# HaydenFaulkner/VidDet

Hardware: AMD Instinct MI355X
Metric: frames/sec (416x416) yolo3_darknet53 fwd+bwd (higher is better)
Workload: dtype f32; 1 GPU; yolo3_darknet53_coco training, batch 64/GPU, 416x416, fp32, fwd+bwd+SGD-momentum (BASELINE configs[2]; the reference trains with SGD, not Adam); classes=80, global_batch=64, parallelism=dp1, hip_graph=False

## Files before the change

### include/viddet_hip.h

```cpp
#ifndef VIDDET_HIP_H
#define VIDDET_HIP_H

#include <stdint.h>

#ifdef __cplusplus
extern "C" {
#endif

#define VD_OK            0
#define VD_EINVAL       -1
#define VD_ELAUNCH      -2
#define VD_EWORKSPACE   -3

#define VD_MAX_TAPS 27

#define VD_EPI_AFFINE    1
#define VD_EPI_LEAKY     2
#define VD_EPI_RESIDUAL  4
#define VD_MATH_SPLIT    16
#define VD_MATH_BF16     32

#define VD_MATH_F16X2    64
#define VD_MATH_NOHALO   128
#define VD_STORE_BF16    256
#define VD_WGRAD_HALO    512
#define VD_CONV_STREAMK  1024
#define VD_CONV_PARITY4  2048
#define VD_CONV_SPLITK   4096
#define VD_SK_MAX_WG        2048
#define VD_SK_HEADER_BYTES  32768
#define VD_SK_SPLIT_CNT_OFF   4096
#define VD_SK_SPLIT_MAX_TILES 4096
#define VD_SK_TIMEOUT_TICKS 4000
#define VD_AMAX_SLOTS    32
#define VD_AMAX_STRIDE   64
#define VD_AMAX_FLOATS   (VD_AMAX_SLOTS * VD_AMAX_STRIDE)

const char* vd_last_error(void);
int vd_version(void);
#define VD_ABI_VERSION 6
int vd_abi_version(void);
int64_t vd_sizeof_desc(int which);

typedef struct {
    const float* in;
    const float* wp;
    float*       out;
    const float* scale;
    const float* shift;
    const float* residual;
    int32_t N, Hi, Wi, Ci;
    int32_t Hg, Wg;
    int32_t in_stride;
    int32_t T;
    int32_t dy[VD_MAX_TAPS], dx[VD_MAX_TAPS];
// ... 11 lines not shown
    float*  stats_part;
    const float* bs_z;
    const float* bs_scale;
    const float* bs_shift;
    const float* bs_mean;
    const float* bs_invstd;
    float*  bs_part;
    float   bs_slope;
    const float* amax_in;
    const float* amax_w;
    float*  amax_out;
    void*   sk_ws;
    int64_t sk_ws_bytes;
    int32_t par_cin;
    int32_t par_mask;
} vd_conv_desc;

int vd_conv_igemm(const vd_conv_desc* d, void* stream);
int vd_conv_igemm_streamk(const vd_conv_desc* d);
int64_t vd_conv_igemm_streamk_ws_bytes(void);
int vd_conv_igemm_mtiles(const vd_conv_desc* d);

int vd_conv_igemm_bf16(const vd_conv_desc* d, int out_f32, void* stream);
int vd_conv_igemm_bf16_streamk(const vd_conv_desc* d, int out_f32);
int vd_conv_igemm_bf16_mtiles(const vd_conv_desc* d);
int vd_pack_weight_bf16(const float* wp_f32, void* wp_bf16, int Co, int Co_pad, int Ci, int Ci_pad, int T,
                        void* stream);
int vd_stem_im2col_bf16(const float* in, void* col, int N, int H, int W, int nchw, void* stream);

typedef struct {
// ... 67 lines not shown
                    const double* sums2, double count, int64_t M, int C, float slope,
                    float* dx, float* amax_out , void* stream);

typedef struct {
    const float* gamma;
    const float* beta;
    const float* scale;
    int32_t C;
    int32_t pad_;
} vd_guard_item;
int vd_range_guard(const vd_guard_item* items, int n, float thresh, float* ratios, int32_t* flags, void* stream);

int vd_amax_merge(const float* a, const float* b, float* out, void* stream);
int vd_amax(const float* x, int64_t n, float* amax, void* stream);
int vd_amax_segments(const float* base, const int64_t* seg, int nseg, float* amax, void* stream);

int vd_add(const float* a, const float* b, float* out, int64_t n, void* stream);
int vd_fill(float* out, float v, int64_t n, void* stream);
int vd_upsample2x_concat(const float* up, const float* route, float* out,
                         int N, int Ho, int Wo, int Cu, int Cr, void* stream);
int vd_upsample2x_concat_bwd(const float* dout, float* dup, float* droute,
                             int N, int Ho, int Wo, int Cu, int Cr, void* stream);
int vd_nchw_to_nhwc(const float* in, float* out, int N, int C, int H, int W, void* stream);
int vd_preprocess_u8_nhwc(const uint8_t* in, float* out, int64_t npix, void* stream);
int vd_preprocess_u8_nchw(const uint8_t* in, float* out, int N, int H, int W, void* stream);
int vd_temporal_pool(const float* x, float* y, int32_t* argmax, int B, int K, int64_t inner, int type,
                     void* stream);
int vd_temporal_pool_bwd(const float* dy, const int32_t* argmax, float* dx, int B, int K,
                         int64_t inner, int type, void* stream);
int vd_frame_slice(const float* x, float* y, int B, int K, int k0, int kc, int64_t inner, int backward, void* stream);
// ... 58 lines not shown
```

### viddet_amd/csrc/vd_conv.hip

```cpp

#include "vd_conv_igemm.h"

int vd_igemm_sk_dispatch(const vd_conv_desc& d, int tile, hipStream_t s);
int vd_igemm_sk_applies(const vd_conv_desc& d, int tile);
int vd_igemm_par_dispatch(const vd_conv_desc& d, int tile, hipStream_t s);
int vd_igemm_par_tile(int tile);
int vd_igemm_par_bm(int tile);

namespace {

int igemm_resolve_tile(const vd_conv_desc& d) {
    int tile = d.tile;
    if (tile <= 0 || tile > 8) {
        if (d.Co <= 32) tile = 7;
        else if (d.Co <= 64) tile = 6;
        else tile = 2;
    }
    return tile;
}

int igemm_tile_bm(int tile) { return (tile == 4 || tile == 5) ? 64 : 128; }

int igemm_split_resolve_tile(const vd_conv_desc& d) {
    int tile = d.tile;
// ... 530 lines not shown
                }
            }
            v[e] = val;
        }
        reinterpret_cast<f32x4*>(col)[i] = v;
    }
}

int check_taps(int T, const int32_t* dy, const int32_t* dx, int Hi, int Wi) {
    if (T < 1 || T > VD_MAX_TAPS) return 0;
    for (int t = 0; t < T; ++t)
        if (dy[t] < -64 || dy[t] > 64 || dx[t] < -64 || dx[t] > 64) return 0;
    return Hi < 4096 && Wi < 4096;
}

}

extern "C" {

#if VD_STAMP
int vd_debug_stamps_f32(unsigned long long* out) {
    return hipMemcpyFromSymbol(out, HIP_SYMBOL(g_stamps_f32), sizeof(unsigned long long) * 16) == hipSuccess ? 0 : 1;
}
#endif

int vd_conv_igemm(const vd_conv_desc* d, void* stream) {
    VD_REQUIRE(d && d->in && d->wp && d->out, "vd_conv_igemm: null pointer");
    VD_REQUIRE(d->Ci > 0 && d->Ci % 32 == 0, "vd_conv_igemm: Ci=%d must be a positive multiple of 32", d->Ci);
    VD_REQUIRE(d->N > 0 && d->Hg > 0 && d->Wg > 0 && d->Co > 0, "vd_conv_igemm: bad shape");
    VD_REQUIRE(check_taps(d->T, d->dy, d->dx, d->Hi, d->Wi), "vd_conv_igemm: bad tap list (T=%d)", d->T);
    VD_REQUIRE(d->Kfr >= 1 && d->Kfr < 128 && d->N % d->Kfr == 0, "vd_conv_igemm: bad Kfr=%d", d->Kfr);
    VD_REQUIRE((d->flags & VD_CONV_PARITY4) || d->ldo >= d->Co, "vd_conv_igemm: ldo < Co");
    VD_REQUIRE((int64_t)d->N * d->Hi * d->Wi < (1ll << 31), "vd_conv_igemm: input pixel count overflows int32");
    VD_REQUIRE((int64_t)d->N * d->Hg * d->Wg < (1ll << 31), "vd_conv_igemm: GEMM row count overflows int32");
    VD_REQUIRE((d->Hg - 1) * d->out_stride + d->out_oy < d->Ho && (d->Wg - 1) * d->out_stride + d->out_ox < d->Wo,
               "vd_conv_igemm: output grid exceeds output tensor");
    VD_REQUIRE(!(d->flags & VD_EPI_RESIDUAL) || (d->residual && (d->ldr >= d->Co || (d->flags & VD_CONV_PARITY4))), "vd_conv_igemm: residual missing");
    VD_REQUIRE((d->in_scale == nullptr) == (d->in_shift == nullptr), "vd_conv_igemm: in_scale/in_shift mismatch");
    VD_REQUIRE(!d->stats_part || (d->flags & 7) == 0, "vd_conv_igemm: fused BN statistics need a raw (epilogue-free) output");
    VD_REQUIRE(!d->bs_part || (!d->stats_part && !d->in_scale && d->bs_z && d->bs_scale && d->bs_shift && d->bs_mean && d->bs_invstd),
               "vd_conv_igemm: fused BN backward reductions need all five bs_* inputs (and no forward statistics / in-load transform)");
    VD_REQUIRE(!(d->flags & VD_CONV_STREAMK) || !d->sk_ws || ((uintptr_t)d->sk_ws % 16 == 0 && d->sk_ws_bytes >= VD_SK_HEADER_BYTES),
               "vd_conv_igemm: VD_CONV_STREAMK workspace must be 16-byte aligned and hold its header");
    VD_REQUIRE(!(d->flags & VD_MATH_F16X2) || (d->amax_in && d->amax_w && !d->in_scale),
               "vd_conv_igemm: VD_MATH_F16X2 needs amax_in and amax_w (and no in-load transform)");
    hipStream_t s = (hipStream_t)stream;
    if (d->flags & VD_CONV_PARITY4) {
        VD_REQUIRE((d->flags & VD_MATH_F16X2) && !(d->flags & (VD_EPI_AFFINE | VD_EPI_LEAKY)) && !d->stats_part && !d->in_scale,
                   "vd_conv_igemm: VD_CONV_PARITY4 runs in VD_MATH_F16X2 with a residual / bs_* epilogue only");
        VD_REQUIRE(d->T == 4 && d->dy[0] == 0 && d->dx[0] == 0 && d->dy[1] == 0 && d->dx[1] == 1 && d->dy[2] == 1 && d->dx[2] == 0 &&
                   d->dy[3] == 1 && d->dx[3] == 1 && d->in_stride == 1 && d->Hg == d->Hi && d->Wg == d->Wi && d->Kfr == 1,
                   "vd_conv_igemm: VD_CONV_PARITY4 taps are the offsets (0,0) (0,1) (1,0) (1,1) on the gradient's own grid");
        VD_REQUIRE(d->out_stride == 2 && d->Ho == 2 * d->Hg && d->Wo == 2 * d->Wg && d->par_cin >= 32 && d->par_cin % 32 == 0 &&
                   d->Co == 4 * d->par_cin && d->ldo >= d->par_cin && d->ldo % 4 == 0 && (uintptr_t)d->out % 16 == 0 &&
                   (!(d->flags & VD_EPI_RESIDUAL) || (d->ldr % 4 == 0 && (uintptr_t)d->residual % 16 == 0)),
                   "vd_conv_igemm: VD_CONV_PARITY4 geometry (even output, Co = 4 par_cin, aligned rows)");
        VD_REQUIRE(!d->bs_part || (((uintptr_t)d->bs_z | (uintptr_t)d->bs_scale | (uintptr_t)d->bs_shift | (uintptr_t)d->bs_mean |
                                    (uintptr_t)d->bs_invstd) % 16 == 0), "vd_conv_igemm: VD_CONV_PARITY4 bs_* alignment");
        vd_igemm_par_dispatch(*d, vd_igemm_par_tile(d->tile), s);
        VD_CHECK_LAUNCH("vd_conv_igemm/parity4");
        return VD_OK;
    }
    if (d->in_scale) dispatch_igemm<true>(*d, s);
    else dispatch_igemm<false>(*d, s);
    VD_CHECK_LAUNCH("vd_conv_igemm");
    return VD_OK;
}

int vd_conv_igemm_streamk(const vd_conv_desc* d) {
    if (!d || !(d->flags & VD_CONV_STREAMK) || !(d->flags & VD_MATH_F16X2)) return 0;
    return vd_igemm_sk_applies(*d, igemm_split_resolve_tile(*d));
}

int64_t vd_conv_igemm_streamk_ws_bytes(void) {
    return (int64_t)VD_SK_HEADER_BYTES + (int64_t)device_cus() * 256 * 256 * 4;
}

int vd_conv_igemm_mtiles(const vd_conv_desc* d) {
    if (!d) return 0;
    const int64_t M = (int64_t)d->N * d->Hg * d->Wg;
// ... 137 lines not shown
```

### viddet_amd/csrc/vd_conv_igemm.h

```cpp
#pragma once
#include "vd_common.h"
#include "vd_wgrad_halo.h"
#include <stdlib.h>

namespace {


#ifndef VD_WG_REMAP
#define VD_WG_REMAP 1
#endif
#ifndef VD_KORDER
#define VD_KORDER 1
#endif
#ifndef VD_SETPRIO
#define VD_SETPRIO 1
#endif
#ifndef VD_PROBE
#define VD_PROBE 0
#endif
#ifndef VD_PD
#define VD_PD 3
#endif
#ifndef VD_BNT
#define VD_BNT 0
// ... 97 lines not shown
template <> struct Terms<2> { static constexpr int N = 3; static constexpr int QA[6] = {1, 0, 0, 0, 0, 0}, QB[6] = {0, 1, 0, 0, 0, 0}; };
template <> struct Terms<1> { static constexpr int N = 1; static constexpr int QA[6] = {0, 0, 0, 0, 0, 0}, QB[6] = {0, 0, 0, 0, 0, 0}; };

__device__ __forceinline__ unsigned udiv_rcp(unsigned n, unsigned d, unsigned rcp) {
    unsigned q = d == 1u ? n : __umulhi(n, rcp);
    q -= (q * d > n) ? 1u : 0u;
    return q;
}

struct RowInfo {
    int64_t off;
    unsigned mask;
};

template <int WM, int WN, int TM, int TN, bool XF, bool SP, bool M16 = false, bool BS = false, int NPL = 3, bool HALO = false, bool SK = false,
          bool PAR = false>
__global__ __launch_bounds__(WM * WN * 64, ((!SP && WM * WN == 8) ? 4 : ((SP && WM * WN == 4) ? 2 : 1))) void k_conv_igemm(const vd_conv_desc p, const int64_t zd_in, const int64_t zd_w, const int sk_lds_flag, const int sk_timeout) {
    static_assert(NPL == 3 || ((NPL == 1 || NPL == 2) && SP), "planes");
    static_assert(!SK || (NPL == 2 && VD_KORDER && !VD_KROT && !XF), "stream-K: the fp16-split tiles, taps-innermost K order");
    static_assert(!PAR || (NPL == 2 && !HALO && !SK && VD_KORDER && !VD_KROT), "parity-fused data gradient: fp16-split tiles, generic loop");
    static_assert(NPL != 2 || !XF, "the fp16 split needs the max-abs of the operand it splits: no in-load transform");
    static_assert(!HALO || (NPL == 2 && WM * WN == 8 && WN * TN * 32 >= 64), "the halo loop exists for the 8-wave fp16-split tiles");
    constexpr int SP_ROWB = NPL * 64;
    constexpr int NTERM = Terms<NPL>::N;
    static_assert(!M16 || SP, "the 16x16x32 shape exists for the bf16 operands of the split arithmetic");
    constexpr int BM = WM * TM * 32, BN = WN * TN * 32;
    constexpr int NT = WM * WN * 64;
    constexpr int RPP = NT / 8;
    constexpr bool BHALF = BN < RPP;
    constexpr int AP = BM / RPP, BP = BHALF ? 1 : BN / RPP;
    static_assert(WM * WN == 4 || WM * WN == 8, "4 or 8 waves");
    static_assert(BM % RPP == 0 && (BHALF || BN % RPP == 0), "tile vs loader");
    static_assert(!BHALF || SP, "the half-populated weight pass exists for the split-math tiles");
    extern __shared__ __attribute__((aligned(16))) float smem[];
    float* As = smem;
    float* Bs = smem + 2 * BM * LDS_LD;
// ... 16 lines not shown
        const int tg0 = g * tq + (g < tr ? g : tr), tgn = tq + (g < tr ? 1 : 0);
        const int64_t U = (int64_t)tgn * upt;
        const int64_t ub = U * j / gs, ue = U * (j + 1) / gs;
        sk_brem = (int)(ub % upt);
        sk_erem = (int)(ue % upt);
        const int tb = (int)(ub / upt), te = (int)(ue / upt);
        sk_tfirst = tg0 + tb;
        sk_t0 = sk_tfirst + (sk_brem ? 1 : 0);
        sk_nwhole = te - (tb + (sk_brem ? 1 : 0));
        if (sk_nwhole < 0) sk_nwhole = 0;
        sk_tlast = tg0 + te;
        sk_nitems = (sk_erem ? 1 : 0) + sk_nwhole + (sk_brem ? 1 : 0);
        sk_me = gbase + j;
    }
    float amx = 0.f;

    int sexp_a = 0, sexp_b = 0;
    float scl_a = 1.f, scl_b = 1.f;
    if (NPL == 2) {
        sexp_a = vd_f16_scale_exp(vd_amax_read(p.amax_in));
        sexp_b = vd_f16_scale_exp(vd_amax_read(p.amax_w));
        scl_a = __uint_as_float((unsigned)(127 + sexp_a) << 23);
        scl_b = __uint_as_float((unsigned)(127 + sexp_b) << 23);
    }

    STAMP(0);
    const int tlane = (int)(threadIdx.x & 63) < p.T ? (int)(threadIdx.x & 63) : 0;
    const int tap_dy = p.dy[tlane], tap_dx = p.dx[tlane], tap_dz = p.dz[tlane];
    const unsigned rcp_w = 0xFFFFFFFFu / (unsigned)p.Wg + 1u, rcp_h = 0xFFFFFFFFu / (unsigned)p.Hg + 1u;

// ... 138 lines not shown
#pragma unroll
                for (int e = 0; e < 4; ++e) {
                    float t = v[e] * sc[e] + sh[e];
                    t = t > 0.f ? t : t * p.in_slope;
                    v[e] = ok ? t : 0.f;
                }
            }
            ra[i] = v;
        }
        const int64_t koff = (int64_t)t_tap * p.Ci + c0;
#pragma unroll
        for (int i = 0; i < BP; ++i) {
            const int64_t o = boff[i] + koff;
            const int64_t sel = (boff[i] >= 0 && !(VD_PROBE & 16)) ? o : zd_w;
#if VD_BNT
            rb[i] = __builtin_nontemporal_load(reinterpret_cast<const f32x4*>(p.wp + sel));
#else
            rb[i] = *reinterpret_cast<const f32x4*>(p.wp + sel);
#endif
        }
#if VD_KORDER
        ++t_tap;
        if (t_tap >= p.T) {
            t_tap = 0;
            c0 += BK;
            if (VD_KROT && c0 >= p.Ci) c0 = 0;
        }
        tap_soff = tap_off(t_tap);
#else
        c0 += BK;
        if (c0 >= p.Ci) {
            c0 = 0;
            ++t_tap;
// ... 7 lines not shown
            const int c = (tid & 7) >> 1, half = (tid & 1) << 3;
            const int oh = ((c ^ key) << 4) + half, ol = (((4 + c) ^ key) << 4) + half;
            char* a3 = As3 + buf * BM * SP_ROWB;
            char* b3 = Bs3 + buf * BN * SP_ROWB;
#pragma unroll
            for (int i = 0; i < AP; ++i) {
                uint2 h, l;
                split2(ra[i], scl_a, h, l);
                char* r = a3 + (lrow + RPP * i) * SP_ROWB;
                *reinterpret_cast<uint2*>(r + oh) = h;
                *reinterpret_cast<uint2*>(r + ol) = l;
            }
#pragma unroll
            for (int i = 0; i < BP; ++i) {
                if (BHALF && lrow >= BN) break;
                uint2 h, l;
                split2(rb[i], scl_b, h, l);
                char* r = b3 + (lrow + RPP * i) * SP_ROWB;
                *reinterpret_cast<uint2*>(r + oh) = h;
                *reinterpret_cast<uint2*>(r + ol) = l;
            }
            return;
        }
        if (SP) {
            const int wkey = M16 ? 2 * ((lrow >> 3) & 1) : ((lrow >> 2) & 3);
            const int wsl = ((((tid & 7) >> 1) ^ wkey) << 4) + ((tid & 1) << 3);
            char* a3 = As3 + buf * BM * SP_ROWB + wsl;
            char* b3 = Bs3 + buf * BN * SP_ROWB + wsl;
#pragma unroll
            for (int i = 0; i < AP; ++i) {
                uint2 h, m, l;
                char* r = a3 + (lrow + RPP * i) * SP_ROWB;
                if (NPL == 3) {
// ... 182 lines not shown
            return *reinterpret_cast<const f32x4*>(p.in + sel);
        };
        auto hstore = [&](const f32x4 v, int c, int s) {
            const int ro_ = (c & 1) * ABUF + (((hvalid >> s) & 1u) ? s * 8192 : hsink);
            uint2 h, l;
            split2(v, scl_a, h, l);
            *reinterpret_cast<uint2*>(Ah + ro_ + hl0) = h;
            *reinterpret_cast<uint2*>(Ah + ro_ + hl1) = l;
        };
        int bt = 0, bc0 = cbeg * BK;
        auto gloadB = [&](f32x4 (&rb)[BP]) {
            const int64_t koff = (int64_t)bt * p.Ci + bc0;
#pragma unroll
            for (int i = 0; i < BP; ++i) {
                const int64_t sel = boff[i] >= 0 ? boff[i] + koff : zd_w;
                rb[i] = *reinterpret_cast<const f32x4*>(p.wp + sel);
            }
            if (++bt >= HT) { bt = 0; bc0 += BK; }
        };
        auto lstoreB = [&](int buf, const f32x4 (&rb)[BP]) {
            const int key = f16x2_key<M16>(lrow);
            const int oh = ((hcs ^ key) << 4) + hhalf, ol = (((4 + hcs) ^ key) << 4) + hhalf;
#pragma unroll
            for (int i = 0; i < BP; ++i) {
                uint2 h, l;
                split2(rb[i], scl_b, h, l);
                char* r = Bh + (buf * BN + lrow + RPP * i) * 128;
                *reinterpret_cast<uint2*>(r + oh) = h;
                *reinterpret_cast<uint2*>(r + ol) = l;
            }
        };
        const int lsel = M16 ? (lane >> 4) : (lane >> 5);
        auto hrows = [&](int (&av)[NRB], int abuf, int tap) {
            const int ro = __builtin_amdgcn_readlane(tap_ro, tap);
#pragma unroll
            for (int b = 0; b < NRB; ++b) {
                const int j = ((amask[b] >> tap) & 1u) ? jbase[b] + ro : ZROW;
                av[b] = abuf * ABUF + j * 128 + ((f16x2_key<M16>(j) ^ lsel) << 4);
            }
        };
        const int swz = f16x2_key<M16>(lane & (RBS - 1));
        auto fragsA = [&](v4i (&fa)[NRB][2], const int (&av)[NRB], int kc) {
// ... 625 lines not shown
    int lds = lds_fixed;
    if (HALO) {
        const int64_t hb = halo_lds_bytes(BM, BN, d.Wi);
        lds = hb > lds_epi ? (int)hb : lds_epi;
    }
    int64_t nblk = vd_cdiv((int64_t)d.N * d.Hg * d.Wg, BM) * vd_cdiv(d.Co, BN);
    int sk_flag_off = 0;
    if (SK) {
        const int G = streamk_grid(d, BM, BN, (SP && WM * WN == 4) ? 2 : 1);
        lds = (lds + 15) & ~15;
        if (G == 0 || lds + 16 > 160 * 1024) return 1;
        sk_flag_off = lds;
        lds += 16;
        nblk = G;
    }
    static bool attr_done = false;
    auto kfn = k_conv_igemm<WM, WN, TM, TN, XF, SP, M16, BS, NPL, HALO, SK, PAR>;
    if (!attr_done) {
        (void)hipFuncSetAttribute(reinterpret_cast<const void*>(kfn), hipFuncAttributeMaxDynamicSharedMemorySize,
                                  HALO ? 160 * 1024 : lds_fixed + (SK ? 16 : 0));
        attr_done = true;
    }
    const float* zp = zero_page();
    const int64_t zd_in = zp - d.in, zd_w = zp - d.wp;
    static const int sk_timeout = getenv("VD_SK_TIMEOUT_TICKS") ? atoi(getenv("VD_SK_TIMEOUT_TICKS")) : VD_SK_TIMEOUT_TICKS;
    hipLaunchKernelGGL(kfn, dim3((unsigned)nblk), dim3(WM * WN * 64), lds, s, d, zd_in, zd_w, sk_flag_off, sk_timeout);
    return 0;
}

}
```

### viddet_amd/lib.py

```python
import ctypes as C
import os

_HERE = os.path.dirname(os.path.abspath(__file__))
LIB_PATH = os.environ.get("VD_LIB") or os.path.join(_HERE, "csrc", "libviddet_hip.so")

ABI_VERSION = 6
VD_MAX_TAPS = 27
EPI_AFFINE, EPI_LEAKY, EPI_RESIDUAL = 1, 2, 4
MATH_SPLIT = 16
MATH_BF16 = 32
MATH_F16X2 = 64
MATH_NOHALO = 128
STORE_BF16 = 256
WGRAD_HALO = 512
CONV_STREAMK = 1024
CONV_SPLITK = 4096
CONV_PARITY4 = 2048
SK_HEADER_BYTES = 32768
AMAX_SLOTS, AMAX_STRIDE = 32, 64
AMAX_FLOATS = AMAX_SLOTS * AMAX_STRIDE

_fp = C.c_void_p


# ... 2 lines not shown
        ("in_", _fp), ("wp", _fp), ("out", _fp), ("scale", _fp), ("shift", _fp), ("residual", _fp),
        ("N", C.c_int32), ("Hi", C.c_int32), ("Wi", C.c_int32), ("Ci", C.c_int32),
        ("Hg", C.c_int32), ("Wg", C.c_int32), ("in_stride", C.c_int32), ("T", C.c_int32),
        ("dy", C.c_int32 * VD_MAX_TAPS), ("dx", C.c_int32 * VD_MAX_TAPS), ("dz", C.c_int32 * VD_MAX_TAPS),
        ("Kfr", C.c_int32),
        ("Ho", C.c_int32), ("Wo", C.c_int32), ("Co", C.c_int32),
        ("out_stride", C.c_int32), ("out_oy", C.c_int32), ("out_ox", C.c_int32),
        ("ldo", C.c_int32), ("ldr", C.c_int32), ("flags", C.c_int32), ("slope", C.c_float),
        ("in_scale", _fp), ("in_shift", _fp), ("in_slope", C.c_float), ("tile", C.c_int32),
        ("stats_part", _fp),
        ("bs_z", _fp), ("bs_scale", _fp), ("bs_shift", _fp), ("bs_mean", _fp), ("bs_invstd", _fp), ("bs_part", _fp),
        ("bs_slope", C.c_float),
        ("amax_in", _fp), ("amax_w", _fp), ("amax_out", _fp),
        ("sk_ws", _fp), ("sk_ws_bytes", C.c_int64),
        ("par_cin", C.c_int32), ("par_mask", C.c_int32),
    ]


class WgradDesc(C.Structure):
    _fields_ = [
        ("in_", _fp), ("dout", _fp), ("dwp", _fp),
        ("N", C.c_int32), ("Hi", C.c_int32), ("Wi", C.c_int32), ("Ci", C.c_int32),
        ("Hg", C.c_int32), ("Wg", C.c_int32), ("Co", C.c_int32), ("ldd", C.c_int32),
        ("in_stride", C.c_int32), ("T", C.c_int32),
        ("dy", C.c_int32 * VD_MAX_TAPS), ("dx", C.c_int32 * VD_MAX_TAPS), ("dz", C.c_int32 * VD_MAX_TAPS),
        ("Kfr", C.c_int32), ("splits", C.c_int32),
        ("in_scale", _fp), ("in_shift", _fp), ("in_slope", C.c_float), ("flags", C.c_int32),
        ("amax_in", _fp), ("amax_dout", _fp),
    ]

# ... 37 lines not shown
    "vd_bn_stats": (_i, [_p, _i64, _i, _p, _p, _i64, _p]),
    "vd_bn_sum_partials_ws_bytes": (_i64, [_i, _i]),
    "vd_bn_sum_partials": (_i, [_p, _i, _i, _p, _p, _i64, _p]),
    "vd_bn_finalize": (_i, [_p, _d, _i, _p, _p, _f, _f, _p, _p, _p, _p, _p, _p, _p]),
    "vd_bn_sum_finalize": (_i, [_p, _i, _i, _p, _d, _p, _p, _f, _f, _p, _p, _p, _p, _p, _p, _p, _i64, _p]),
    "vd_bn_sum_param_grads": (_i, [_p, _i, _i, _p, _p, _p, _p, _i64, _p]),
    "vd_bn_fold_eval": (_i, [_p, _p, _p, _p, _f, _i, _p, _p, _p]),
    "vd_bn_apply_leaky": (_i, [_p, _p, _p, _p, _p, _i64, _i, _f, _p, _p]),
    "vd_bn_bwd_reduce": (_i, [_p, _p, _p, _p, _p, _p, _i64, _i, _f, _p, _p, _i64, _p]),
    "vd_bn_param_grads": (_i, [_p, _i, _p, _p, _p]),
    "vd_bn_bwd_apply": (_i, [_p, _p, _p, _p, _p, _p, _p, _d, _i64, _i, _f, _p, _p, _p]),
    "vd_range_guard": (_i, [_p, _i, _f, _p, _p, _p]),
    "vd_amax": (_i, [_p, _i64, _p, _p]),
    "vd_amax_segments": (_i, [_p, _p, _i, _p, _p]),
    "vd_amax_merge": (_i, [_p, _p, _p, _p]),
    "vd_add": (_i, [_p, _p, _p, _i64, _p]),
    "vd_fill": (_i, [_p, _f, _i64, _p]),
    "vd_upsample2x_concat": (_i, [_p, _p, _p, _i, _i, _i, _i, _i, _p]),
    "vd_upsample2x_concat_bwd": (_i, [_p, _p, _p, _i, _i, _i, _i, _i, _p]),
    "vd_nchw_to_nhwc": (_i, [_p, _p, _i, _i, _i, _i, _p]),
    "vd_stem_conv_blocks": (_i, [_i, _i, _i]),
    "vd_stem_conv": (_i, [_p, _p, _p, _i, _i, _i, _i, _p, _p, C.c_float, _i, _i, _p, _p]),
    "vd_stem_conv_c32_bf16": (_i, [_p, _p, _p, _p, C.c_float, C.POINTER(ConvDesc), _p]),
    "vd_stem_wgrad_ws_bytes": (_i64, [_i, _i, _i]),
    "vd_stem_wgrad": (_i, [_p, _p, _i, _p, _i, _i, _i, _p, _i64, _p]),
    "vd_preprocess_u8_nhwc": (_i, [_p, _p, _i64, _p]),
    "vd_preprocess_u8_nchw": (_i, [_p, _p, _i, _i, _i, _p]),
    "vd_temporal_pool": (_i, [_p, _p, _p, _i, _i, _i64, _i, _p]),
    "vd_temporal_pool_bwd": (_i, [_p, _p, _p, _i, _i, _i64, _i, _p]),
    "vd_temporal_cat": (_i, [_p, _p, _i, _i, _i64, _i, _i, _p]),
# ... 68 lines not shown
```

### viddet_amd/model.py

```python
import ctypes as C
import math
import re
from collections import OrderedDict

import numpy as np
import torch

from . import lib as L
from . import ops
from .lib import ConvDesc, WgradDesc, EPI_AFFINE, EPI_LEAKY, EPI_RESIDUAL
from .ops import round_up, fwd_taps, dgrad_plans

from .consts import ANCHORS, STRIDES, BN_EPS, BN_MOMENTUM, LEAKY_SLOPE


class Slot:

    def __init__(self):
        self.value = None


class Program:

    def __init__(self):
# ... 116 lines not shown
            return None
        return str(torch.cuda.get_device_properties(torch.cuda.current_device()).gcnArchName).split(":")[0]

    def _read_file(self):
        import ast
        import json
        import os
        out = {}
        p = self.path()
        if p is None or not os.path.exists(p):
            return out
        try:
            doc = json.load(open(p))
            if doc.get("library") not in (None, self.library_id()):
                return out
            arch = self.device_arch()
            if arch is not None and doc.get("device") not in (None, arch):
                return out
            for k, v in doc.get("entries", {}).items():
                out[ast.literal_eval(k)] = tuple(v) if isinstance(v, list) else v
        except (OSError, ValueError, SyntaxError) as e:
            print("viddet_amd: ignoring tuning table %s (%s)" % (p, e), flush=True)
            return {}
        return out

    def load(self):
        import os
        self._loaded = True
        world = self._world()
        self._synced_world = world
# ... 633 lines not shown
        self.process_group = process_group
        self._training = False
        self._recording = False
        self._programs = {}
        self._sk_ws = {}
        self._range_exact = set()
        self._fold_dirty = True
        self._stats_version = 1
        self._weights_version = 1
        self._pack_stream = None
        self._pack_event = None
        self._graph_cache = {}
        self.use_graphs = False
        import os as _os
        self.overlap_wgrad = _os.environ.get('VD_OVERLAP', '1') != '0'
        self.fuse_bn_stats = _os.environ.get('VD_FUSE_STATS', '1') != '0'
        self.precision = 'fp32'
        self.bucketed_allreduce = _os.environ.get('VD_BUCKETED', '1') != '0'
        self.alias_skip_grad = _os.environ.get('VD_ALIAS_SKIP', '1') != '0'
        self.fuse_bn_bwd = _os.environ.get('VD_FUSE_BWD', '1') != '0'
        self.bucket_elems = int(float(_os.environ.get('VD_BUCKET_MB', '32')) * (1 << 18))
        self._pending_reduces = []
        self._reduced_from = 1 << 62
        self._dp_stats = {'buckets': 0, 'bucket_bytes': 0}
        self._bucket_group = None
        self._build(len(self._classes))

    def _build(self, num_class):
        self.num_class = num_class
        self.nodes, self.tensors, self.head_names = build_graph(num_class, self._k, self._k_join_type,
# ... 22 lines not shown
        dev = self.device
        self.weights = torch.zeros(off, device=dev)
        self.grads = torch.zeros(off, device=dev)
        self.momentum_buf = torch.zeros(off, device=dev)
        soff = 0
        for n in self.conv_nodes:
            if n.bn:
                n.stat_off = soff
                soff += 2 * round_up(n.cout, 64)
        self.running = torch.zeros(max(soff, 1), device=dev)
        self._wamax = torch.zeros(len(self.conv_nodes) * L.AMAX_FLOATS, device=dev)
        self._wamax_seg = torch.tensor([[n.w_off, n.w_numel] for n in self.conv_nodes], dtype=torch.int64, device=dev)
        for i, n in enumerate(self.conv_nodes):
            n.wamax = self._wamax[i * L.AMAX_FLOATS:(i + 1) * L.AMAX_FLOATS]
        self._wamax_dirty = True
        self.aux = torch.zeros(max(1, sum(6 * round_up(n.cout, 64) for n in self.conv_nodes if n.bn)), device=dev)
        self.sums = torch.zeros(max(1, sum(4 * round_up(n.cout, 64) for n in self.conv_nodes)), dtype=torch.float64,
                                device=dev)
        aoff = doff = 0
        for n in self.conv_nodes:
            c64 = round_up(n.cout, 64)
            if n.bn:
                v = self.aux[aoff:aoff + 6 * c64]
                n.fold_scale, n.fold_shift = v[0:n.cout], v[c64:c64 + n.cout]
                n.b_scale, n.b_shift = v[2 * c64:2 * c64 + n.cout], v[3 * c64:3 * c64 + n.cout]
                n.b_mean, n.b_invstd = v[4 * c64:4 * c64 + n.cout], v[5 * c64:5 * c64 + n.cout]
                aoff += 6 * c64
            n.sums = self.sums[doff:doff + 2 * c64]
            n.sums2 = self.sums[doff + 2 * c64:doff + 4 * c64]
            doff += 4 * c64
# ... 147 lines not shown
                    out[-1][1] = hi
                else:
                    out.append([lo, hi, p.lr_mult, p.wd_mult])
            self._opt_ranges = [tuple(r) for r in out]
        return self._opt_ranges

    def _params_changed(self):
        self._fold_dirty = True
        self._weights_version += 1
        self._wamax_dirty = True

    def _refresh_wamax(self):
        if self._wamax_dirty:
            L.check(L.load().vd_amax_segments(self.weights.data_ptr(), self._wamax_seg.data_ptr(), len(self.conv_nodes),
                                              self._wamax.data_ptr(), L.stream_ptr()), 'vd_amax_segments')
            self._wamax_dirty = False

    def _buffers(self, key, B, H, W, train):
        ck = ('buf', B, H, W, train)
        if ck in self._programs:
            return self._programs[ck]
        dev = self.device
        bufs = {}
        for name, (c, div, ld, fr) in self.tensors.items():
            if name == 'in':
                bufs['in'] = torch.empty(B * fr, 3, H, W, device=dev)
                continue
            bufs[name] = torch.empty(B * fr, H // div, W // div, ld, device=dev)
        if self.noback:
            for nm, c_, d_ in ROUTE_TENSORS:
                bufs['in:' + nm] = torch.empty(B, c_, H // d_, W // d_, device=dev)
# ... 46 lines not shown
        d.Ho, d.Wo, d.Co = Ho, Wo, n.co_pad
        d.out_stride, d.out_oy, d.out_ox = 1, 0, 0
        d.ldo = d.ldr = n.co_pad
        flags = 0
        if scale is not None or shift is not None:
            flags |= EPI_AFFINE
            d.scale = scale.data_ptr() if scale is not None else None
            d.shift = shift.data_ptr() if shift is not None else None
        if leaky:
            flags |= EPI_LEAKY
        if residual is not None:
            flags |= EPI_RESIDUAL
            d.residual = residual.data_ptr()
        d.flags, d.slope = flags, LEAKY_SLOPE
        d.amax_in, d.amax_w = self._amax_or_none(bufs, n.src), n.wamax.data_ptr()
        self._set_streamk(d, 0)
        if amax_out:
            d.amax_out = bufs['amax:' + n.dst].data_ptr()
        return d

    def _amax_or_none(self, bufs, name):
        if name in self._range_exact:
            return None
        return bufs['amax:' + name].data_ptr()

    def check_operand_ranges(self, thresh=2.0 ** -16):
        bn = [n for n in self.conv_nodes if n.bn]
        if not bn:
            return {}
        if getattr(self, '_guard', None) is None:
# ... 530 lines not shown
        last_side = [None]

        def ev_record(e, on_side):
            def f():
                e.record(side if on_side else torch.cuda.current_stream())
            return f

        def ev_wait(e, on_side):
            def f():
                (side if on_side else torch.cuda.current_stream()).wait_event(e)
            return f

        bucket_hi, bucket_acc = [self.n_weight], [0]
        written = set(self.head_names)
        dgrad_packs = []

        alias = {}
        producers = {m.dst: m for m in self.conv_nodes if m.bn}
        consumers = {}
        for m in self.nodes:
            srcs = [m.src, m.residual] if isinstance(m, ConvNode) else ([m.up, m.route] if isinstance(m, UpcatNode) else
                                                                          ([m.a, m.b] if isinstance(m, AddNode) else [m.src]))
            for t in srcs:
                if t:
                    consumers.setdefault(t, []).append(m)
        fused_bwd = set()
        tgrad = {t: False for t in self.tensors}
        for m in self.nodes:
            if isinstance(m, ConvNode):
                tgrad[m.dst] = any(self._node_trainable(m)) or tgrad[m.src] or bool(m.residual and tgrad[m.residual])
# ... 191 lines not shown
            res_src = alias.pop(n.src) if n.src in alias else dsrc
            plans = dgrad_plans(n.k, n.pad, n.stride, Hi, Wi, n.kd, n.pad_d)
            pm = producers.get(n.src)
            fuse_m = pm if (self.fuse_bn_bwd and pm is not None and (len(plans) == 1 or (n.kd == 1 and _fuse_bwd_s2())) and
                            consumers[n.src][0] is n and pm.fr == n.fr) else None
            bs_rows = 0
            import os as _os
            fused_s2 = (len(plans) == 4 and n.k == 3 and n.stride == 2 and n.pad == 1 and n.kd == 1 and Hi % 2 == 0 and Wi % 2 == 0 and
                        _os.environ.get('VD_S2_FUSED', '1') == '1' and n.cin % 32 == 0 and
                        n.cin <= int(_os.environ.get('VD_S2_FUSED_MAX_CIN', '64')) and
                        self._amax_or_none(bufs, 'dz:' + n.name) is not None and
                        (fp32_math() == 'split2' or (fp32_math() == 'auto' and _os.environ.get('VD_AUTOTUNE', '1') != '0')))
            if fused_s2:
                wp4 = torch.empty(16 * n.cin * n.co_pad, device=dev)
                dgrad_packs.append((n, dict(fused_s2=True), wp4))
                d = ConvDesc()
                d.in_, d.wp, d.out = dz.data_ptr(), wp4.data_ptr(), dsrc.data_ptr()
                d.N, d.Hi, d.Wi, d.Ci = B * n.fr, Ho, Wo, n.co_pad
                d.Hg, d.Wg, d.in_stride = Ho, Wo, 1
                ops._set_taps(d, ops.PARITY4_TAPS)
                d.Kfr, d.Ho, d.Wo, d.Co = 1, Hi, Wi, 4 * n.cin
                d.out_stride, d.out_oy, d.out_ox = 2, 0, 0
                d.ldo = d.ldr = n.cin
                d.par_cin, d.par_mask = n.cin, ops.PARITY4_MASK
                d.flags, d.slope = (EPI_RESIDUAL if acc else 0) | L.MATH_F16X2 | L.CONV_PARITY4, LEAKY_SLOPE
                d.amax_in, d.amax_w = self._amax_or_none(bufs, 'dz:' + n.name), n.wamax.data_ptr()
                if acc:
                    d.residual = res_src.data_ptr()
                seg.hold(d, wp4)
                if fuse_m is not None:
                    d.bs_z = bufs['z:' + fuse_m.dst].data_ptr()
                    d.bs_scale, d.bs_shift = fuse_m.b_scale.data_ptr(), fuse_m.b_shift.data_ptr()
                    d.bs_mean, d.bs_invstd = fuse_m.b_mean.data_ptr(), fuse_m.b_invstd.data_ptr()
                    d.bs_part, d.bs_slope = stats_ws.data_ptr(), LEAKY_SLOPE
                autotune_desc(d)
                if fuse_m is not None:
                    mt = L.load().vd_conv_igemm_mtiles(C.byref(d))
                    assert mt * 2 * fuse_m.cout * 4 <= stats_ws.numel() * 4, "stats workspace too small"
                    seg.add('vd_fill', stats_ws.data_ptr(), 0.0, mt * 2 * fuse_m.cout)
                seg.add('vd_conv_igemm', C.byref(d), meta=dict(
                    kind='dgrad', node=n.name, k=n.k, stride=n.stride, fused_s2=True,
                    flops=2.0 * n.cin * n.cout * 9 * Ho * Wo * B * n.fr, bytes=self._flops(n, B, H, W, 'dgrad')['bytes']))
                if fuse_m is not None:
                    seg.add('vd_bn_sum_param_grads', stats_ws.data_ptr(), mt, fuse_m.cout, fuse_m.sums2.data_ptr(),
# ... 1 lines not shown
                    fused_bwd.add(fuse_m.name)
                continue
            NF = B * n.fr
            nchunks = 1
            chunk_mb = float(__import__('os').environ.get('VD_S2_CHUNK_MB', '0'))
            if len(plans) == 4 and n.kd == 1 and chunk_mb > 0:
                dz_mb = 4.0 * NF * Ho * Wo * n.co_pad / 1e6
                nchunks = max(1, min(NF, int(math.ceil(dz_mb / chunk_mb))))
            fchunk = (NF + nchunks - 1) // nchunks
            nchunks = (NF + fchunk - 1) // fchunk
            wpks = []
            for plan in plans:
                assert plan['taps'], "a parity class without taps would leave its gradient unwritten"
                wpk = torch.empty(n.cin * len(plan['taps']) * n.co_pad, device=dev)
                dgrad_packs.append((n, plan, wpk))
                wpks.append(wpk)
            in_img, out_img = Ho * Wo * n.co_pad * 4, Hi * Wi * n.cin * 4
            for ch in range(nchunks):
              f0 = ch * fchunk
              fn_ = min(NF, f0 + fchunk) - f0
              par = None
              if _parity_streams() and len(plans) == 4 and self.overlap_wgrad:
                if getattr(self, '_par_streams', None) is None:
                    self._par_streams = [torch.cuda.Stream() for _ in range(3)]
                par = self._par_streams
                e_fork = torch.cuda.Event()
                seg.add_py(lambda e=e_fork: e.record(torch.cuda.current_stream()))
                for st in par:
                    seg.add_py(lambda e=e_fork, st=st: st.wait_event(e))
              for pi, plan in enumerate(plans):
                wpk = wpks[pi]
                d = ConvDesc()
                d.in_, d.wp, d.out = dz.data_ptr() + f0 * in_img, wpk.data_ptr(), dsrc.data_ptr() + f0 * out_img
                d.N, d.Hi, d.Wi, d.Ci = fn_, Ho, Wo, n.co_pad
                d.Hg, d.Wg, d.in_stride = plan['Hg'], plan['Wg'], 1
                ops._set_taps(d, plan['taps'])
                d.Kfr = n.fr if n.kd > 1 else 1
                d.Ho, d.Wo, d.Co = Hi, Wi, n.cin
                d.out_stride, d.out_oy, d.out_ox = n.stride, plan['py'], plan['px']
                d.ldo = d.ldr = n.cin
                d.flags, d.slope = (EPI_RESIDUAL if acc else 0), LEAKY_SLOPE
                d.amax_in, d.amax_w = self._amax_or_none(bufs, 'dz:' + n.name), n.wamax.data_ptr()
                self._set_streamk(d, pi if (par is not None) else 0)
                if acc:
                    d.residual = res_src.data_ptr() + f0 * out_img
                seg.hold(d, wpk)
                nplans = n.stride * n.stride
                if fuse_m is not None:
                    d.bs_z = bufs['z:' + fuse_m.dst].data_ptr() + f0 * out_img
                    d.bs_scale, d.bs_shift = fuse_m.b_scale.data_ptr(), fuse_m.b_shift.data_ptr()
                    d.bs_mean, d.bs_invstd = fuse_m.b_mean.data_ptr(), fuse_m.b_invstd.data_ptr()
                    d.bs_part, d.bs_slope = stats_ws.data_ptr() + bs_rows * 2 * fuse_m.cout * 4, LEAKY_SLOPE
                    autotune_desc(d)
                    bs_rows += L.load().vd_conv_igemm_mtiles(C.byref(d))
                    mt = bs_rows
                    assert mt * 2 * fuse_m.cout * 4 <= stats_ws.numel() * 4, "stats workspace too small"
                seg.add('vd_conv_igemm', C.byref(d), meta=dict(
                    kind='dgrad', node=n.name, k=n.k, stride=n.stride,
                    flops=2.0 * n.cin * n.cout * len(plan['taps']) * plan['Hg'] * plan['Wg'] * fn_,
                    bytes=self._flops(n, B, H, W, 'dgrad')['bytes'] / nplans * fn_ / NF),
                    stream=(par[pi - 1] if (par is not None and pi > 0) else None))
# ... 2 lines not shown
                        e_join = torch.cuda.Event()
                        seg.add_py(lambda e=e_join, st=st: e.record(st))
                        seg.add_py(lambda e=e_join: torch.cuda.current_stream().wait_event(e))
                if fuse_m is not None and pi == len(plans) - 1 and ch == nchunks - 1:
                    seg.add('vd_bn_sum_param_grads', stats_ws.data_ptr(), mt, fuse_m.cout, fuse_m.sums2.data_ptr(),
                            fuse_m.ggamma.data_ptr(), fuse_m.gbeta.data_ptr(), ws.data_ptr(), ws_bytes)
                    fused_bwd.add(fuse_m.name)
        if side is not None and last_side[0] is not None:
            seg.add_py(ev_wait(last_side[0], False))
        seg.hold(ws_w, side, stats_ws)
        bwd.append(seg)
        for sg in fwd + bwd:
            if isinstance(sg, Program):
                autotune_program(sg)
        _TUNE_CACHE.save()
        return dict(fwd=fwd, bwd=bwd, bufs=bufs, slots=slots, losses=losses, dgrad_packs=dgrad_packs, ws=ws)


    def set_storage(self, storage):
        if storage not in ('fp32', 'bf16'):
            raise ValueError("storage must be 'fp32' or 'bf16'")
        if storage == 'bf16' and (self._k > 1 or self.noback or self.temporal_out or getattr(self, 'temporal_side', False)):
            raise NotImplementedError("bf16-storage training is built for the single-frame yolo3_darknet53 network")
        self.storage = storage

    def _tune_bf16_desc(self, d, of32):
        import os
        if os.environ.get("VD_AUTOTUNE", "1") == "0":
            return
        base = d.flags & ~(L.MATH_NOHALO | L.CONV_STREAMK)
        key = ('bf16', d.N, d.Hi, d.Wi, d.Ci, d.Hg, d.Wg, d.in_stride, d.T, d.Co, base, of32, d.out_stride, bool(d.stats_part),
# ... 361 lines not shown

    def _ones(self, c):
        if not hasattr(self, '_const'):
            self._const = (torch.ones(1024, device=self.device), torch.zeros(1024, device=self.device))
        return self._const[0]

    def _zeros(self, c):
        self._ones(c)
        return self._const[1]

    def _refresh_dgrad(self, tp, overlap=False):
        if tp.get('storage') == 'bf16':
            return self._refresh_train_bf16(tp, overlap)
        if tp.get('dgrad_version') == self._weights_version:
            return
        ev = None
        if overlap and self.overlap_wgrad:
            if self._pack_stream is None:
                self._pack_stream = torch.cuda.Stream()
            cur = torch.cuda.current_stream()
            self._pack_stream.wait_stream(cur)
            with torch.cuda.stream(self._pack_stream):
                for n, plan, wpk in tp['dgrad_packs']:
                    self._pack_dgrad(n, plan, wpk)
                ev = torch.cuda.Event()
                ev.record(self._pack_stream)
        else:
            for n, plan, wpk in tp['dgrad_packs']:
                self._pack_dgrad(n, plan, wpk)
        self._pack_event = ev
        tp['dgrad_version'] = self._weights_version

    @staticmethod
    def _pack_dgrad(n, plan, wpk):
        if plan.get('fused_s2'):
            ops.pack_weight_dgrad_s2(n.wp, wpk, Co=n.co_pad, Co_pad=n.co_pad, Ci=n.cin)
        else:
            ops.pack_weight_dgrad(n.wp, wpk, Co=n.co_pad, Co_pad=n.co_pad, Ci=n.cin, kd=n.kd, kh=n.k, kw=n.k,
                                  tap_ids=plan['tap_ids'], src_packed=True)

    @staticmethod
    def _run_segments(segs):
        for s in segs:
            if isinstance(s, Program):
# ... 221 lines not shown
```

Baseline: 1049 frames/s.

## Pre-split conv weights into fp16 hi/lo image once per weight update

Adds a kernel that converts each conv weight tensor, and each packed data-gradient weight, into a pre-split fp16x2 hi/lo image once per weight version, scaled from the weight amax. The igemm kernel gains a WPS template path that loads this image and stores it straight into LDS, skipping the per-tile split2 on the B operand. The work removed is the split arithmetic repeated by every workgroup that reads the same weight tile. In exchange it adds a second weight-sized buffer, an extra split pass after each optimizer step, and new template instantiations. It also relies on the image's byte layout matching the LDS swizzle.

```diff
diff --git a/include/viddet_hip.h b/include/viddet_hip.h
--- a/include/viddet_hip.h
+++ b/include/viddet_hip.h
@@ -38,7 +38,7 @@
 
 const char* vd_last_error(void);
 int vd_version(void);
-#define VD_ABI_VERSION 6
+#define VD_ABI_VERSION 7
 int vd_abi_version(void);
 int64_t vd_sizeof_desc(int which);
 
@@ -80,6 +80,7 @@
     int64_t sk_ws_bytes;
     int32_t par_cin;
     int32_t par_mask;
+    const void* wp_f16x2;
 } vd_conv_desc;
 
 int vd_conv_igemm(const vd_conv_desc* d, void* stream);
@@ -177,6 +178,7 @@
 int vd_amax_merge(const float* a, const float* b, float* out, void* stream);
 int vd_amax(const float* x, int64_t n, float* amax, void* stream);
 int vd_amax_segments(const float* base, const int64_t* seg, int nseg, float* amax, void* stream);
+int vd_split_weight_f16x2_segments(const int64_t* seg, int nseg, void* stream);
 
 int vd_add(const float* a, const float* b, float* out, int64_t n, void* stream);
 int vd_fill(float* out, float v, int64_t n, void* stream);
diff --git a/viddet_amd/csrc/vd_conv.hip b/viddet_amd/csrc/vd_conv.hip
--- a/viddet_amd/csrc/vd_conv.hip
+++ b/viddet_amd/csrc/vd_conv.hip
@@ -568,6 +568,23 @@
     return Hi < 4096 && Wi < 4096;
 }
 
+__global__ void k_split_weight_f16x2(const int64_t* __restrict__ seg) {
+    const int64_t* sg = seg + 4 * blockIdx.y;
+    const float* src = reinterpret_cast<const float*>(sg[0]);
+    char* img = reinterpret_cast<char*>(sg[1]);
+    const int64_t n = sg[2] & ~31ll;
+    const int sexp = vd_f16_scale_exp(vd_amax_read(reinterpret_cast<const float*>(sg[3])));
+    const float scl = __uint_as_float((unsigned)(127 + sexp) << 23);
+    for (int64_t e0 = 8 * ((int64_t)blockIdx.x * blockDim.x + threadIdx.x); e0 < n; e0 += 8ll * gridDim.x * blockDim.x) {
+        char* g = img + (e0 >> 5) * 128 + (e0 & 31) * 2;
+        uint2 ha, la, hb, lb;
+        split2(*reinterpret_cast<const f32x4*>(src + e0), scl, ha, la);
+        split2(*reinterpret_cast<const f32x4*>(src + e0 + 4), scl, hb, lb);
+        *reinterpret_cast<uint4*>(g) = make_uint4(ha.x, ha.y, hb.x, hb.y);
+        *reinterpret_cast<uint4*>(g + 64) = make_uint4(la.x, la.y, lb.x, lb.y);
+    }
+}
+
 }
 
 extern "C" {
@@ -598,6 +615,7 @@
                "vd_conv_igemm: VD_CONV_STREAMK workspace must be 16-byte aligned and hold its header");
     VD_REQUIRE(!(d->flags & VD_MATH_F16X2) || (d->amax_in && d->amax_w && !d->in_scale),
                "vd_conv_igemm: VD_MATH_F16X2 needs amax_in and amax_w (and no in-load transform)");
+    VD_REQUIRE((uintptr_t)d->wp_f16x2 % 16 == 0, "vd_conv_igemm: wp_f16x2 must be 16-byte aligned");
     hipStream_t s = (hipStream_t)stream;
     if (d->flags & VD_CONV_PARITY4) {
         VD_REQUIRE((d->flags & VD_MATH_F16X2) && !(d->flags & (VD_EPI_AFFINE | VD_EPI_LEAKY)) && !d->stats_part && !d->in_scale,
@@ -618,6 +636,13 @@
     if (d->in_scale) dispatch_igemm<true>(*d, s);
     else dispatch_igemm<false>(*d, s);
     VD_CHECK_LAUNCH("vd_conv_igemm");
+    return VD_OK;
+}
+
+int vd_split_weight_f16x2_segments(const int64_t* seg, int nseg, void* stream) {
+    VD_REQUIRE(seg && nseg > 0 && nseg < 65536, "vd_split_weight_f16x2_segments: bad args");
+    hipLaunchKernelGGL(k_split_weight_f16x2, dim3(32, nseg), dim3(256), 0, (hipStream_t)stream, seg);
+    VD_CHECK_LAUNCH("vd_split_weight_f16x2_segments");
     return VD_OK;
 }
 
diff --git a/viddet_amd/csrc/vd_conv_igemm.h b/viddet_amd/csrc/vd_conv_igemm.h
--- a/viddet_amd/csrc/vd_conv_igemm.h
+++ b/viddet_amd/csrc/vd_conv_igemm.h
@@ -135,12 +135,13 @@
 };
 
 template <int WM, int WN, int TM, int TN, bool XF, bool SP, bool M16 = false, bool BS = false, int NPL = 3, bool HALO = false, bool SK = false,
-          bool PAR = false>
+          bool PAR = false, bool WPS = false>
 __global__ __launch_bounds__(WM * WN * 64, ((!SP && WM * WN == 8) ? 4 : ((SP && WM * WN == 4) ? 2 : 1))) void k_conv_igemm(const vd_conv_desc p, const int64_t zd_in, const int64_t zd_w, const int sk_lds_flag, const int sk_timeout) {
     static_assert(NPL == 3 || ((NPL == 1 || NPL == 2) && SP), "planes");
     static_assert(!SK || (NPL == 2 && VD_KORDER && !VD_KROT && !XF), "stream-K: the fp16-split tiles, taps-innermost K order");
     static_assert(!PAR || (NPL == 2 && !HALO && !SK && VD_KORDER && !VD_KROT), "parity-fused data gradient: fp16-split tiles, generic loop");
     static_assert(NPL != 2 || !XF, "the fp16 split needs the max-abs of the operand it splits: no in-load transform");
+    static_assert(!WPS || NPL == 2, "the pre-split weight image exists for the fp16-split arithmetic");
     static_assert(!HALO || (NPL == 2 && WM * WN == 8 && WN * TN * 32 >= 64), "the halo loop exists for the 8-wave fp16-split tiles");
     constexpr int SP_ROWB = NPL * 64;
     constexpr int NTERM = Terms<NPL>::N;
@@ -187,6 +188,7 @@
         sk_me = gbase + j;
     }
     float amx = 0.f;
+    const float* wsrc = WPS ? reinterpret_cast<const float*>(p.wp_f16x2) : p.wp;
 
     int sexp_a = 0, sexp_b = 0;
     float scl_a = 1.f, scl_b = 1.f;
@@ -355,9 +357,9 @@
             const int64_t o = boff[i] + koff;
             const int64_t sel = (boff[i] >= 0 && !(VD_PROBE & 16)) ? o : zd_w;
 #if VD_BNT
-            rb[i] = __builtin_nontemporal_load(reinterpret_cast<const f32x4*>(p.wp + sel));
+            rb[i] = __builtin_nontemporal_load(reinterpret_cast<const f32x4*>(wsrc + sel));
 #else
-            rb[i] = *reinterpret_cast<const f32x4*>(p.wp + sel);
+            rb[i] = *reinterpret_cast<const f32x4*>(wsrc + sel);
 #endif
         }
 #if VD_KORDER
@@ -395,9 +397,13 @@
 #pragma unroll
             for (int i = 0; i < BP; ++i) {
                 if (BHALF && lrow >= BN) break;
+                char* r = b3 + (lrow + RPP * i) * SP_ROWB;
+                if (WPS) {
+                    *reinterpret_cast<f32x4*>(r + (((tid & 7) ^ key) << 4)) = rb[i];
+                    continue;
+                }
                 uint2 h, l;
                 split2(rb[i], scl_b, h, l);
-                char* r = b3 + (lrow + RPP * i) * SP_ROWB;
                 *reinterpret_cast<uint2*>(r + oh) = h;
                 *reinterpret_cast<uint2*>(r + ol) = l;
             }
@@ -610,7 +616,7 @@
 #pragma unroll
             for (int i = 0; i < BP; ++i) {
                 const int64_t sel = boff[i] >= 0 ? boff[i] + koff : zd_w;
-                rb[i] = *reinterpret_cast<const f32x4*>(p.wp + sel);
+                rb[i] = *reinterpret_cast<const f32x4*>(wsrc + sel);
             }
             if (++bt >= HT) { bt = 0; bc0 += BK; }
         };
@@ -619,9 +625,13 @@
             const int oh = ((hcs ^ key) << 4) + hhalf, ol = (((4 + hcs) ^ key) << 4) + hhalf;
 #pragma unroll
             for (int i = 0; i < BP; ++i) {
+                char* r = Bh + (buf * BN + lrow + RPP * i) * 128;
+                if (WPS) {
+                    *reinterpret_cast<f32x4*>(r + (((tid & 7) ^ key) << 4)) = rb[i];
+                    continue;
+                }
                 uint2 h, l;
                 split2(rb[i], scl_b, h, l);
-                char* r = Bh + (buf * BN + lrow + RPP * i) * 128;
                 *reinterpret_cast<uint2*>(r + oh) = h;
                 *reinterpret_cast<uint2*>(r + ol) = l;
             }
@@ -1277,15 +1287,20 @@
         lds += 16;
         nblk = G;
     }
-    static bool attr_done = false;
-    auto kfn = k_conv_igemm<WM, WN, TM, TN, XF, SP, M16, BS, NPL, HALO, SK, PAR>;
-    if (!attr_done) {
+    static bool attr_done[2] = {false, false};
+    const bool wps = NPL == 2 && d.wp_f16x2 != nullptr;
+    auto kfn = k_conv_igemm<WM, WN, TM, TN, XF, SP, M16, BS, NPL, HALO, SK, PAR, false>;
+    if constexpr (NPL == 2) {
+        if (wps) kfn = k_conv_igemm<WM, WN, TM, TN, XF, SP, M16, BS, NPL, HALO, SK, PAR, true>;
+    }
+    if (!attr_done[wps]) {
         (void)hipFuncSetAttribute(reinterpret_cast<const void*>(kfn), hipFuncAttributeMaxDynamicSharedMemorySize,
                                   HALO ? 160 * 1024 : lds_fixed + (SK ? 16 : 0));
-        attr_done = true;
+        attr_done[wps] = true;
     }
     const float* zp = zero_page();
-    const int64_t zd_in = zp - d.in, zd_w = zp - d.wp;
+    const float* wbase = wps ? reinterpret_cast<const float*>(d.wp_f16x2) : d.wp;
+    const int64_t zd_in = zp - d.in, zd_w = zp - wbase;
     static const int sk_timeout = getenv("VD_SK_TIMEOUT_TICKS") ? atoi(getenv("VD_SK_TIMEOUT_TICKS")) : VD_SK_TIMEOUT_TICKS;
     hipLaunchKernelGGL(kfn, dim3((unsigned)nblk), dim3(WM * WN * 64), lds, s, d, zd_in, zd_w, sk_flag_off, sk_timeout);
     return 0;
diff --git a/viddet_amd/lib.py b/viddet_amd/lib.py
--- a/viddet_amd/lib.py
+++ b/viddet_amd/lib.py
@@ -4,7 +4,7 @@
 _HERE = os.path.dirname(os.path.abspath(__file__))
 LIB_PATH = os.environ.get("VD_LIB") or os.path.join(_HERE, "csrc", "libviddet_hip.so")
 
-ABI_VERSION = 6
+ABI_VERSION = 7
 VD_MAX_TAPS = 27
 EPI_AFFINE, EPI_LEAKY, EPI_RESIDUAL = 1, 2, 4
 MATH_SPLIT = 16
@@ -40,6 +40,7 @@
         ("amax_in", _fp), ("amax_w", _fp), ("amax_out", _fp),
         ("sk_ws", _fp), ("sk_ws_bytes", C.c_int64),
         ("par_cin", C.c_int32), ("par_mask", C.c_int32),
+        ("wp_f16x2", _fp),
     ]
 
 
@@ -107,6 +108,7 @@
     "vd_amax": (_i, [_p, _i64, _p, _p]),
     "vd_amax_segments": (_i, [_p, _p, _i, _p, _p]),
     "vd_amax_merge": (_i, [_p, _p, _p, _p]),
+    "vd_split_weight_f16x2_segments": (_i, [_p, _i, _p]),
     "vd_add": (_i, [_p, _p, _p, _i64, _p]),
     "vd_fill": (_i, [_p, _f, _i64, _p]),
     "vd_upsample2x_concat": (_i, [_p, _p, _p, _i, _i, _i, _i, _i, _p]),
diff --git a/viddet_amd/model.py b/viddet_amd/model.py
--- a/viddet_amd/model.py
+++ b/viddet_amd/model.py
@@ -154,6 +154,9 @@
             doc = json.load(open(p))
             if doc.get("library") not in (None, self.library_id()):
                 return out
+            if "entries_from" in doc:
+                src = json.load(open(os.path.join(os.path.dirname(p), os.path.basename(doc["entries_from"]))))
+                doc = dict(doc, entries=src.get("entries", {}))
             arch = self.device_arch()
             if arch is not None and doc.get("device") not in (None, arch):
                 return out
@@ -817,6 +820,7 @@
         self.use_graphs = False
         import os as _os
         self.overlap_wgrad = _os.environ.get('VD_OVERLAP', '1') != '0'
+        self.w_presplit = _os.environ.get('VD_W_PRESPLIT', '1') != '0'
         self.fuse_bn_stats = _os.environ.get('VD_FUSE_STATS', '1') != '0'
         self.precision = 'fp32'
         self.bucketed_allreduce = _os.environ.get('VD_BUCKETED', '1') != '0'
@@ -869,6 +873,12 @@
         for i, n in enumerate(self.conv_nodes):
             n.wamax = self._wamax[i * L.AMAX_FLOATS:(i + 1) * L.AMAX_FLOATS]
         self._wamax_dirty = True
+        self._wimg, self._wimg_seg = None, None
+        if self.w_presplit:
+            self._wimg = torch.zeros(self.n_weight, device=dev)
+            for n in self.conv_nodes:
+                n.wimg = self._wimg[n.w_off:n.w_off + n.w_numel]
+            self._wimg_seg = self._split_table([(self.weights[n.w_off:n.w_off + n.w_numel], n.wimg, n) for n in self.conv_nodes])
         self.aux = torch.zeros(max(1, sum(6 * round_up(n.cout, 64) for n in self.conv_nodes if n.bn)), device=dev)
         self.sums = torch.zeros(max(1, sum(4 * round_up(n.cout, 64) for n in self.conv_nodes)), dtype=torch.float64,
                                 device=dev)
@@ -1046,7 +1056,19 @@
         if self._wamax_dirty:
             L.check(L.load().vd_amax_segments(self.weights.data_ptr(), self._wamax_seg.data_ptr(), len(self.conv_nodes),
                                               self._wamax.data_ptr(), L.stream_ptr()), 'vd_amax_segments')
+            if self._wimg_seg is not None:
+                self._split_weights(self._wimg_seg)
             self._wamax_dirty = False
+
+    def _split_table(self, rows):
+        assert all(src.numel() % 32 == 0 and img.numel() == src.numel() for src, img, _ in rows)
+        t = [[src.data_ptr(), img.data_ptr(), src.numel(), n.wamax.data_ptr()] for src, img, n in rows]
+        return torch.tensor(t, dtype=torch.int64, device=self.device)
+
+    @staticmethod
+    def _split_weights(table):
+        L.check(L.load().vd_split_weight_f16x2_segments(table.data_ptr(), table.shape[0], L.stream_ptr()),
+                'vd_split_weight_f16x2_segments')
 
     def _buffers(self, key, B, H, W, train):
         ck = ('buf', B, H, W, train)
@@ -1123,6 +1145,8 @@
             d.residual = residual.data_ptr()
         d.flags, d.slope = flags, LEAKY_SLOPE
         d.amax_in, d.amax_w = self._amax_or_none(bufs, n.src), n.wamax.data_ptr()
+        if self._wimg is not None:
+            d.wp_f16x2 = n.wimg.data_ptr()
         self._set_streamk(d, 0)
         if amax_out:
             d.amax_out = bufs['amax:' + n.dst].data_ptr()
@@ -1683,6 +1707,14 @@
         bucket_hi, bucket_acc = [self.n_weight], [0]
         written = set(self.head_names)
         dgrad_packs = []
+        dgrad_imgs = []
+
+        def dgrad_image(n, wpk):
+            if self._wimg is None or self._amax_or_none(bufs, 'dz:' + n.name) is None:
+                return None
+            img = torch.zeros_like(wpk)
+            dgrad_imgs.append((wpk, img, n))
+            return img
 
         alias = {}
         producers = {m.dst: m for m in self.conv_nodes if m.bn}
@@ -1904,6 +1936,7 @@
             if fused_s2:
                 wp4 = torch.empty(16 * n.cin * n.co_pad, device=dev)
                 dgrad_packs.append((n, dict(fused_s2=True), wp4))
+                wimg4 = dgrad_image(n, wp4)
                 d = ConvDesc()
                 d.in_, d.wp, d.out = dz.data_ptr(), wp4.data_ptr(), dsrc.data_ptr()
                 d.N, d.Hi, d.Wi, d.Ci = B * n.fr, Ho, Wo, n.co_pad
@@ -1915,9 +1948,11 @@
                 d.par_cin, d.par_mask = n.cin, ops.PARITY4_MASK
                 d.flags, d.slope = (EPI_RESIDUAL if acc else 0) | L.MATH_F16X2 | L.CONV_PARITY4, LEAKY_SLOPE
                 d.amax_in, d.amax_w = self._amax_or_none(bufs, 'dz:' + n.name), n.wamax.data_ptr()
+                if wimg4 is not None:
+                    d.wp_f16x2 = wimg4.data_ptr()
                 if acc:
                     d.residual = res_src.data_ptr()
-                seg.hold(d, wp4)
+                seg.hold(d, wp4, wimg4)
                 if fuse_m is not None:
                     d.bs_z = bufs['z:' + fuse_m.dst].data_ptr()
                     d.bs_scale, d.bs_shift = fuse_m.b_scale.data_ptr(), fuse_m.b_shift.data_ptr()
@@ -1949,7 +1984,7 @@
                 assert plan['taps'], "a parity class without taps would leave its gradient unwritten"
                 wpk = torch.empty(n.cin * len(plan['taps']) * n.co_pad, device=dev)
                 dgrad_packs.append((n, plan, wpk))
-                wpks.append(wpk)
+                wpks.append((wpk, dgrad_image(n, wpk)))
             in_img, out_img = Ho * Wo * n.co_pad * 4, Hi * Wi * n.cin * 4
             for ch in range(nchunks):
               f0 = ch * fchunk
@@ -1964,7 +1999,7 @@
                 for st in par:
                     seg.add_py(lambda e=e_fork, st=st: st.wait_event(e))
               for pi, plan in enumerate(plans):
-                wpk = wpks[pi]
+                wpk, wimg = wpks[pi]
                 d = ConvDesc()
                 d.in_, d.wp, d.out = dz.data_ptr() + f0 * in_img, wpk.data_ptr(), dsrc.data_ptr() + f0 * out_img
                 d.N, d.Hi, d.Wi, d.Ci = fn_, Ho, Wo, n.co_pad
@@ -1976,10 +2011,12 @@
                 d.ldo = d.ldr = n.cin
                 d.flags, d.slope = (EPI_RESIDUAL if acc else 0), LEAKY_SLOPE
                 d.amax_in, d.amax_w = self._amax_or_none(bufs, 'dz:' + n.name), n.wamax.data_ptr()
+                if wimg is not None:
+                    d.wp_f16x2 = wimg.data_ptr()
                 self._set_streamk(d, pi if (par is not None) else 0)
                 if acc:
                     d.residual = res_src.data_ptr() + f0 * out_img
-                seg.hold(d, wpk)
+                seg.hold(d, wpk, wimg)
                 nplans = n.stride * n.stride
                 if fuse_m is not None:
                     d.bs_z = bufs['z:' + fuse_m.dst].data_ptr() + f0 * out_img
@@ -2012,7 +2049,8 @@
             if isinstance(sg, Program):
                 autotune_program(sg)
         _TUNE_CACHE.save()
-        return dict(fwd=fwd, bwd=bwd, bufs=bufs, slots=slots, losses=losses, dgrad_packs=dgrad_packs, ws=ws)
+        return dict(fwd=fwd, bwd=bwd, bufs=bufs, slots=slots, losses=losses, dgrad_packs=dgrad_packs, ws=ws,
+                    dgrad_split=self._split_table(dgrad_imgs) if dgrad_imgs else None)
 
 
     def set_storage(self, storage):
@@ -2404,6 +2442,7 @@
             return self._refresh_train_bf16(tp, overlap)
         if tp.get('dgrad_version') == self._weights_version:
             return
+        self._refresh_wamax()
         ev = None
         if overlap and self.overlap_wgrad:
             if self._pack_stream is None:
@@ -2413,11 +2452,15 @@
             with torch.cuda.stream(self._pack_stream):
                 for n, plan, wpk in tp['dgrad_packs']:
                     self._pack_dgrad(n, plan, wpk)
+                if tp.get('dgrad_split') is not None:
+                    self._split_weights(tp['dgrad_split'])
                 ev = torch.cuda.Event()
                 ev.record(self._pack_stream)
         else:
             for n, plan, wpk in tp['dgrad_packs']:
                 self._pack_dgrad(n, plan, wpk)
+            if tp.get('dgrad_split') is not None:
+                self._split_weights(tp['dgrad_split'])
         self._pack_event = ev
         tp['dgrad_version'] = self._weights_version
 
```

Result: no change. 1058 frames/s (median of 6 runs) (+0.8%).
